# gareth-cross/mini_opt

Hardware: AMD Instinct MI355X
Metric: batched dense KKT Newton steps/sec, n=64 fp64 (higher is better)
Workload: dtype f64; 1 GPU; BASELINE configs[2]: batch=65536 per GPU, n=64 / 8 eq / 32 box, m_r=128, J-level input (row-major J), one mo_newton_step launch per step; mode=step, kernel=fused_mfma_f64_n64, batch_per_gpu=65536, batch_total=65536, n=64, k=8, m=32, m_r=128, parallelism=batch-sharded x1, no collectives

## Files before the change

### mini_opt_amd/csrc/kkt_fused.hip

```cpp
#include <math.h>
#include <stdlib.h>

#include <type_traits>

#include "mo_fused_select.h"

namespace mo {
namespace {

typedef double d2 __attribute__((ext_vector_type(2)));
typedef double d4 __attribute__((ext_vector_type(4)));

#ifdef MO_FUSED_STAMPS
#define MO_STAMP(i)                                                                                   \
  do {                                                                                                \
    __builtin_amdgcn_sched_barrier(0);                                                                \
    unsigned long long t__;                                                                           \
    asm volatile("s_memtime %0\n\ts_waitcnt lgkmcnt(0)" : "=s"(t__)::"memory");                       \
    stamp_acc[i] += t__ - stamp_prev;                                                                 \
    stamp_prev = t__;                                                                                 \
    __builtin_amdgcn_sched_barrier(0);                                                                \
  } while (0)
#else
#define MO_STAMP(i) do { } while (0)
// ... 188 lines not shown
        if (ta == tb && r > j) { row = 16 * ta + r; col = 16 * ta + j; }
        U[ta * NB + tb][t] = (row < nn && col < nn) ? G[row + (size_t)col * ld] : 0.0;
      }
    }
    cvec[ta] = (16 * ta + j < nn) ? cg[16 * ta + j] : 0.0;
  }
}

__device__ inline int lane_id() {
  int l;
  asm volatile("v_mbcnt_lo_u32_b32 %0, -1, 0\n\tv_mbcnt_hi_u32_b32 %0, -1, %0" : "=v"(l));
  return l;
}

typedef const KernelArgs __attribute__((address_space(4)))* KArgs;
__device__ inline KArgs fresh_args() {
  KArgs p = (KArgs)__builtin_amdgcn_kernarg_segment_ptr();
  asm volatile("" : "+s"(p));
  return p;
}

__device__ inline void dma16(const void* gsrc, unsigned lds_dst) {
  unsigned keep;
  asm volatile(
      "s_mov_b32 %0, m0\n\ts_mov_b32 m0, %2\n\ts_nop 0\n\tglobal_load_lds_dwordx4 %1, off\n\ts_mov_b32 m0, %0"
      : "=&s"(keep)
      : "v"(gsrc), "s"(lds_dst)
      : "memory");
}
__device__ inline const void* uniform_ptr(const void* p) {
  const unsigned long long b = (unsigned long long)(uintptr_t)p;
  const unsigned lo = __builtin_amdgcn_readfirstlane((unsigned)b), hi = __builtin_amdgcn_readfirstlane((unsigned)(b >> 32));
  return (const void*)(uintptr_t)(((unsigned long long)hi << 32) | lo);
}
#ifdef MO_J_NO_NT
#define MO_J_POLICY ""
#else
#define MO_J_POLICY " nt"
#endif
template <int IMM> __device__ inline void dma16_s(const void* sbase_in, unsigned voff, unsigned lds_dst_in) {
  const void* sbase = uniform_ptr(sbase_in);
  const unsigned lds_dst = __builtin_amdgcn_readfirstlane(lds_dst_in);
  unsigned keep;
  asm volatile(
      "s_mov_b32 %0, m0\n\ts_mov_b32 m0, %3\n\ts_nop 0\n\tglobal_load_lds_dwordx4 %1, %2 offset:%4" MO_J_POLICY "\n\ts_mov_b32 m0, %0"
      : "=&s"(keep)
      : "v"(voff), "s"(sbase), "s"(lds_dst), "i"(IMM)
      : "memory");
}
__device__ inline void dma4_s(const void* sbase_in, unsigned voff, unsigned lds_dst_in) {
  const void* sbase = uniform_ptr(sbase_in);
  const unsigned lds_dst = __builtin_amdgcn_readfirstlane(lds_dst_in);
  unsigned keep;
  asm volatile(
      "s_mov_b32 %0, m0\n\ts_mov_b32 m0, %3\n\ts_nop 0\n\tglobal_load_lds_dword %1, %2\n\ts_mov_b32 m0, %0"
      : "=&s"(keep)
      : "v"(voff), "s"(sbase), "s"(lds_dst)
      : "memory");
}
__device__ inline void dma4(const void* gsrc, unsigned lds_dst) {
  unsigned keep;
  asm volatile(
      "s_mov_b32 %0, m0\n\ts_mov_b32 m0, %2\n\ts_nop 0\n\tglobal_load_lds_dword %1, off\n\ts_mov_b32 m0, %0"
      : "=&s"(keep)
      : "v"(gsrc), "s"(lds_dst)
      : "memory");
}
__device__ inline void dma_doubles(const double* src, unsigned lds_dst, int count, int lane) {
  const unsigned voff = 4u * (unsigned)lane;
  if (lane < 2 * count) dma4_s(src, voff, lds_dst);
  if (lane + 64 < 2 * count) dma4_s(reinterpret_cast<const char*>(src) + 256, voff, lds_dst + 256);
  if (count > 64) {
    if (lane + 128 < 2 * count) dma4_s(reinterpret_cast<const char*>(src) + 512, voff, lds_dst + 512);
    if (lane + 192 < 2 * count) dma4_s(reinterpret_cast<const char*>(src) + 768, voff, lds_dst + 768);
  }
  if (count > 128) {
#pragma unroll
    for (int c = 4; c < 8; ++c)
      if (lane + 64 * c < 2 * count) dma4_s(reinterpret_cast<const char*>(src) + 256 * c, voff, lds_dst + 256 * c);
  }
}
template <int N> __device__ inline void wait_vmcnt() { asm volatile("s_waitcnt vmcnt(%0)" ::"i"(N) : "memory"); }
__device__ inline void lds_fence() { asm volatile("s_waitcnt lgkmcnt(0)" ::: "memory"); }

#ifdef MO_MASKED_PAD_4
#define MO_MASKED_PAD "4"
#else
#define MO_MASKED_PAD "0"
#endif
template <int LANE_IN_ROW> __device__ inline double row_bcast64(double v) {
  return __longlong_as_double(__builtin_amdgcn_mov_dpp(__double_as_longlong(v), 0x150 + LANE_IN_ROW, 0xf, 0xf, false));
}
template <unsigned long long MASK> __device__ inline void masked_set(double& dst, double src) {
  unsigned long long save;
  asm volatile("s_mov_b64 %[sv], exec\n\ts_mov_b32 exec_lo, %[lo]\n\ts_mov_b32 exec_hi, %[hi]\n\tv_mov_b64 %[d], %[s]\n\t"
               "s_mov_b64 exec, %[sv]\n\ts_nop " MO_MASKED_PAD
               : [d] "+v"(dst), [sv] "=&s"(save)
               : [s] "v"(src), [lo] "i"((unsigned)(MASK & 0xffffffffull)), [hi] "i"((unsigned)(MASK >> 32)));
}
template <unsigned long long MASK> __device__ inline void masked_set_neg(double& dst, double src) {
  unsigned long long save;
  asm volatile("s_mov_b64 %[sv], exec\n\ts_mov_b32 exec_lo, %[lo]\n\ts_mov_b32 exec_hi, %[hi]\n\tv_max_f64 %[d], -%[s], -%[s]\n\t"
               "s_mov_b64 exec, %[sv]\n\ts_nop " MO_MASKED_PAD
               : [d] "+v"(dst), [sv] "=&s"(save)
               : [s] "v"(src), [lo] "i"((unsigned)(MASK & 0xffffffffull)), [hi] "i"((unsigned)(MASK >> 32)));
}
template <unsigned long long MASK> __device__ inline void masked_zero4(d4& T) {
  unsigned long long save;
  double t0 = T[0], t1 = T[1], t2 = T[2], t3 = T[3];
  asm volatile(
      "s_mov_b64 %[sv], exec\n\ts_mov_b32 exec_lo, %[lo]\n\ts_mov_b32 exec_hi, %[hi]\n\tv_mov_b64 %[a], 0\n\tv_mov_b64 %[b], 0\n\t"
      "v_mov_b64 %[c], 0\n\tv_mov_b64 %[d], 0\n\ts_mov_b64 exec, %[sv]\n\ts_nop " MO_MASKED_PAD
      : [a] "+v"(t0), [b] "+v"(t1), [c] "+v"(t2), [d] "+v"(t3), [sv] "=&s"(save)
      : [lo] "i"((unsigned)(MASK & 0xffffffffull)), [hi] "i"((unsigned)(MASK >> 32)));
  T[0] = t0; T[1] = t1; T[2] = t2; T[3] = t3;
}
template <int K>
__device__ inline void sweep_step_lean(d4& T, double& bad, int g, int j) {
  constexpr int src_g = K & 3, src_t = K >> 2;
  constexpr unsigned long long mcol = 0x0001000100010001ull << K;
  constexpr unsigned long long mrow = 0xFFFFull << (16 * src_g);
  const double rowreg = T[src_t];
  const double d = readlane_f64(rowreg, 16 * src_g + K);
  double inv = __builtin_amdgcn_rcp(d);
  inv = fma(inv, fma(-d, inv, 1.0), inv);
  asm volatile("v_fma_f64 %0, %1, 0, %0" : "+v"(bad) : "v"(inv));
#ifdef MO_SWEEP_VALU_ROW
  double rk = bcast_from_row<src_g>(rowreg) * inv;
#else
  double rk = bpermute_f64((16 * src_g + j) * 4, rowreg) * inv;
#endif
  masked_set_neg<mcol>(rk, inv);
  double f[4];
#pragma unroll
  for (int t = 0; t < 4; ++t) f[t] = row_bcast64<K>(T[t]);
  masked_zero4<mcol>(T);
#pragma unroll
  for (int t = 0; t < 4; ++t) T[t] = fma(-f[t], rk, T[t]);
  double rowk_new = T[src_t];
  masked_set<mrow>(rowk_new, rk);
  T[src_t] = rowk_new;
}
template <int K, int KEND> struct SweepLoop {
  static __device__ inline void run(d4& T, double& bad, int npiv, int g, int j) {
    if (K < npiv) sweep_step_lean<K>(T, bad, g, j);
    SweepLoop<K + 1, KEND>::run(T, bad, npiv, g, j);
  }
};
template <int KEND> struct SweepLoop<KEND, KEND> {
  static __device__ inline void run(d4&, double&, int, int, int) {}
};
__device__ inline bool sweep_tile(d4& T, int npiv, int g, int j) {
  double bad = 0.0;
  SweepLoop<0, 16>::run(T, bad, npiv, g, j);
  return bad == 0.0;
}

template <int NT, int D, int JMODE = JMODE_VECTOR, int NY = 1, bool ROW0 = true>
struct JStream {
  static constexpr bool FLAT = JMODE == JMODE_FLAT, GATHER = JMODE == JMODE_GATHER;
  static constexpr int N = 16 * NT, NB = NT + NY, NH = NT / 2, NI = GATHER ? 2 * NT : (FLAT ? N / 8 : NH), DPS = NI + 1, SLOT = NH * 1024 + 64;
  static_assert((D - 1) * DPS <= 63, "vmcnt is a 6-bit counter");
  static_assert(D >= 2 && D <= 8, "ring depth");
  const char* jbase;
  const char* rbase;
  unsigned joff, roff;
  unsigned jstep;
  const double* tail_j; const double* tail_r; int rem, row_len, g_, j_;
  bool act0, act1, act2, act3;
  const char* lane_piece;
  const char* r_elem;
  unsigned ring_base;
  int lane, nsteps;
  long long rs_, cs_;

  __device__ inline void init(const double* Jp, const double* rg, const char* smem, unsigned ring_base_, int lane_, int g, int j, int m_r,
                              int nn = N, long long rs = -1, long long cs = 1) {
    if (rs < 0) rs = nn;
    jbase = reinterpret_cast<const char*>(Jp);
    rbase = reinterpret_cast<const char*>(rg);
    rs_ = 8 * rs; cs_ = 8 * cs;
    joff = GATHER ? (unsigned)(g * rs_ + 2 * j * cs_) : (unsigned)(g * nn + 2 * j) * 8u;
    jstep = GATHER ? (unsigned)(4 * rs_) : 32u * (unsigned)nn;
    act0 = 2 * j < nn; act1 = 32 + 2 * j < nn; act2 = 64 + 2 * j < nn; act3 = 96 + 2 * j < nn;
    roff = 4u * (unsigned)lane_;
    lane_piece = smem + lane_ * 16;
    r_elem = smem + NH * 1024 + 8 * g;
    ring_base = ring_base_; lane = lane_; nsteps = m_r >> 2;
    rem = m_r & 3; row_len = nn; g_ = g; j_ = j;
    tail_j = Jp + (size_t)(4 * nsteps) * (GATHER ? rs : (long long)nn); tail_r = rg + 4 * nsteps;
  }
  template <int IMM> __device__ static inline void dma4_si(const void* sbase_in, unsigned voff, unsigned lds_dst_in) {
    const void* sbase = uniform_ptr(sbase_in);
    const unsigned lds_dst = __builtin_amdgcn_readfirstlane(lds_dst_in);
    unsigned keep;
    asm volatile(
        "s_mov_b32 %0, m0\n\ts_mov_b32 m0, %3\n\ts_nop 0\n\tglobal_load_lds_dword %1, %2 offset:%4\n\ts_mov_b32 m0, %0"
        : "=&s"(keep)
        : "v"(voff), "s"(sbase), "s"(lds_dst), "i"(IMM)
        : "memory");
  }
  template <int SL> __device__ inline void issue() {
    const unsigned dst = ring_base + SL * SLOT;
    if (GATHER) {
#pragma unroll
      for (int c = 0; c < NT; ++c) {
        const int col0 = 32 * (c >> 1) + (c & 1);
        if (col0 < row_len) {
          const char* sb = jbase + (long long)col0 * cs_;
          if (col0 + 2 * j_ < row_len) { dma4_si<0>(sb, joff, dst + 512 * c); dma4_si<4>(sb, joff, dst + 512 * c + 256 - 4); }
        } else {
          if (lane == 0) { dma4_si<0>(jbase, 0u, dst + NH * 1024 + 48); dma4_si<0>(jbase, 0u, dst + NH * 1024 + 48); }
        }
      }
      if (lane < 8) dma4_s(rbase, roff, dst + NH * 1024);
      jbase += jstep;
      rbase += 32;
      return;
    }
    if (FLAT) {
      const int run = 32 * row_len;
#pragma unroll
      for (int i = 0; i < NI; ++i) {
        if (256 * i < run) {
          if (256 * i + 4 * lane < run) dma4_s(jbase + 256 * i, 4u * (unsigned)lane, dst + 256 * i);
        } else {
          if (lane == 0) dma4_s(jbase, 0u, dst + NH * 1024 + 48);
        }
      }
      if (lane < 8) dma4_s(rbase, roff, dst + NH * 1024);
      jbase += jstep;
      rbase += 32;
      return;
    }
    if (act0) dma16_s<0>(jbase, joff, dst);
    if (NH > 1 && act1) dma16_s<256>(jbase, joff, dst + 1024 - 256);
    if (NH > 2 && act2) dma16_s<512>(jbase, joff, dst + 2048 - 512);
    if (NH > 3 && act3) dma16_s<768>(jbase, joff, dst + 3072 - 768);
    if (lane < 8) dma4_s(rbase, roff, dst + NH * 1024);
    jbase += jstep;
    rbase += 32;
  }
  __device__ inline void wait_for_oldest(int younger) const {
    if (younger >= D - 1) { wait_vmcnt<(D - 1) * DPS>(); return; }
    switch (younger) {
      case 0: wait_vmcnt<0>(); break;
      case 1: wait_vmcnt<1 * DPS>(); break;
      case 2: wait_vmcnt<(D > 2 ? 2 : 0) * DPS>(); break;
      case 3: wait_vmcnt<(D > 3 ? 3 : 0) * DPS>(); break;
      case 4: wait_vmcnt<(D > 4 ? 4 : 0) * DPS>(); break;
      case 5: wait_vmcnt<(D > 5 ? 5 : 0) * DPS>(); break;
      default: wait_vmcnt<(D > 6 ? 6 : 0) * DPS>(); break;
    }
  }
  double rsq;
  template <int SL, bool RSQ = false> __device__ inline void consume(int q, d4 (&U)[NB * NB], double (&cpart)[NT]) {
    wait_for_oldest(nsteps - 1 - q);
    double ops[NT];
    if (GATHER) {
      const int* src = reinterpret_cast<const int*>(lane_piece - lane * 16 + SL * SLOT) + lane;
#pragma unroll
      for (int c = 0; c < NT; ++c) ops[c] = __hiloint2double(src[128 * c + 64], src[128 * c]);
    } else if (FLAT) {
      const double* src = reinterpret_cast<const double*>(lane_piece - lane * 16 + SL * SLOT) + g_ * row_len + 2 * j_;
#pragma unroll
      for (int h = 0; h < NH; ++h) {
        const double v0 = src[32 * h], v1 = src[32 * h + 1];
        ops[2 * h] = (32 * h + 2 * j_ < row_len) ? v0 : 0.0;
        ops[2 * h + 1] = (32 * h + 2 * j_ + 1 < row_len) ? v1 : 0.0;
      }
    } else {
#pragma unroll
      for (int h = 0; h < NH; ++h) {
        const d2 v = *(const d2*)(lane_piece + SL * SLOT + h * 1024);
        ops[2 * h] = v[0]; ops[2 * h + 1] = v[1];
      }
    }
    const double rq = *(const double*)(r_elem + SL * SLOT);
    lds_fence();
    if (q + D < nsteps) issue<SL>();
    if (RSQ) rsq = fma(rq, rq, rsq);
#pragma unroll
    for (int ta = 0; ta < NT; ++ta) {
      cpart[ta] = fma(ops[ta], rq, cpart[ta]);
#pragma unroll
      for (int tb = ta; tb < NT; ++tb) jtj_mfma(U[ta * NB + tb], ops[ta], ops[tb], ta);
    }
  }
#ifdef MO_ROW0_ALL_NY
  static constexpr bool ROW0_VGPR = NT == 8 && ROW0;
#elif !defined(MO_NO_ROW0_VGPR)
  static constexpr bool ROW0_VGPR = NT == 8 && NY == 1 && ROW0;
#else
  static constexpr bool ROW0_VGPR = false;
#endif
#ifndef MO_ROW0_ASM_QUAL
#define MO_ROW0_ASM_QUAL
#endif
#ifndef MO_ROW0_PREFIX
#define MO_ROW0_PREFIX "s_nop 3\n\t"
#endif
  __device__ static inline void jtj_mfma(d4& acc, double a, double b, int ta) {
    if (ROW0_VGPR && ta == 0) asm MO_ROW0_ASM_QUAL (MO_ROW0_PREFIX "v_mfma_f64_16x16x4_f64 %0, %1, %2, %0" : "+v"(acc) : "v"(a), "v"(b));
    else acc = __builtin_amdgcn_mfma_f64_16x16x4f64(a, b, acc, 0, 0, 0);
  }
  __device__ static inline void finish() {
    if (ROW0_VGPR) asm volatile("s_nop 15\n\ts_nop 3" ::: "memory");
  }
#define MO_FOR_SLOTS(F) F(0) F(1) F(2) F(3) F(4) F(5) F(6) F(7)
  __device__ inline void prologue() {
#define MO_ISSUE(u) if (u < D && u < nsteps) issue<(u < D ? u : 0)>();
    MO_FOR_SLOTS(MO_ISSUE)
#undef MO_ISSUE
  }
  template <bool RSQ = false>
  __device__ inline void run(d4 (&U)[NB * NB], double (&cpart)[NT]) {
    if (RSQ) rsq = 0.0;
    for (int q0 = 0; q0 < nsteps; q0 += D) {
#define MO_CONSUME(u) if (u < D && q0 + u < nsteps) consume<(u < D ? u : 0), RSQ>(q0 + u, U, cpart);
      MO_FOR_SLOTS(MO_CONSUME)
#undef MO_CONSUME
    }
    if (rem) {
      double ops[NT];
#pragma unroll
      for (int c = 0; c < NT; ++c) ops[c] = 0.0;
      double rq = 0.0;
      if (g_ < rem) {
        if (GATHER) {
          const char* row = reinterpret_cast<const char*>(tail_j) + g_ * rs_ + 2 * j_ * cs_;
#pragma unroll
          for (int c = 0; c < NT; ++c) {
            const int col0 = 32 * (c >> 1) + (c & 1);
            if (col0 + 2 * j_ < row_len) ops[c] = *reinterpret_cast<const double*>(row + (long long)col0 * cs_);
          }
        } else {
          const double* row = tail_j + (size_t)g_ * row_len + 2 * j_;
#pragma unroll
          for (int h = 0; h < NH; ++h) {
            if (32 * h + 2 * j_ < row_len) ops[2 * h] = row[32 * h];
            if (32 * h + 2 * j_ + 1 < row_len) ops[2 * h + 1] = row[32 * h + 1];
          }
        }
        rq = tail_r[g_];
      }
      if (RSQ) rsq = fma(rq, rq, rsq);
#pragma unroll
      for (int ta = 0; ta < NT; ++ta) {
        cpart[ta] = fma(ops[ta], rq, cpart[ta]);
#pragma unroll
        for (int tb = ta; tb < NT; ++tb) jtj_mfma(U[ta * NB + tb], ops[ta], ops[tb], ta);
      }
    }
    finish();
  }
#undef MO_FOR_SLOTS
};

template <int NT, int NY> __device__ inline int tile_pivots(int pa, int k) { return pa < NT + NY - 1 ? 16 : k - 16 * (NY - 1); }
template <int NT, int NY = 1>
__device__ inline bool block_eliminate(d4 (&U)[(NT + NY) * (NT + NY)], int k, int g, int j) {
  constexpr int NB = NT + NY;
  bool ok = true;
#pragma unroll
  for (int pa = 0; pa < NB; ++pa) {
    ok = sweep_tile(U[pa * NB + pa], tile_pivots<NT, NY>(pa, k), g, j) && ok;
    __builtin_amdgcn_sched_barrier(0);
#pragma unroll
    for (int pc = pa + 1; pc < NB; ++pc) {
      d4 negZ = mfma4(U[pa * NB + pa], U[pa * NB + pc], d4{0.0, 0.0, 0.0, 0.0});
#pragma unroll
      for (int pb = pa + 1; pb <= pc; ++pb) U[pb * NB + pc] = mfma4(U[pa * NB + pb], negZ, U[pb * NB + pc]);
      __builtin_amdgcn_sched_barrier(0);
    }
  }
  return ok;
}

#ifndef MO_LA_MIN_NT
#define MO_LA_MIN_NT 6
#endif
template <int NB> constexpr int la_count(int pa) { int c = 0; for (int pc = pa + 2; pc < NB; ++pc) c += 1 + (pc - pa); return c; }
template <int NB> constexpr int la_pc(int pa, int idx) {
  for (int pc = pa + 2; pc < NB; ++pc) { const int n = 1 + (pc - pa); if (idx < n) return pc; idx -= n; }
  return -1;
}
template <int NB> constexpr int la_sub(int pa, int idx) {
  for (int pc = pa + 2; pc < NB; ++pc) { const int n = 1 + (pc - pa); if (idx < n) return idx; idx -= n; }
  return -1;
}
template <int NT, int PA, int IDX, int Q> __device__ inline void la_mfma(d4 (&U)[(NT + 1) * (NT + 1)], d4& negZ) {
  constexpr int NB = NT + 1;
  if constexpr (IDX < la_count<NB>(PA)) {
    constexpr int pc = la_pc<NB>(PA, IDX), sub = la_sub<NB>(PA, IDX);
    if constexpr (sub == 0) {
      if constexpr (Q == 0) negZ = d4{0.0, 0.0, 0.0, 0.0};
      negZ = __builtin_amdgcn_mfma_f64_16x16x4f64(U[PA * NB + PA][Q], U[PA * NB + pc][Q], negZ, 0, 0, 0);
    } else {
      U[(PA + sub) * NB + pc] = __builtin_amdgcn_mfma_f64_16x16x4f64(U[PA * NB + (PA + sub)][Q], negZ[Q], U[(PA + sub) * NB + pc], 0, 0, 0);
    }
  }
}
template <int NB> constexpr int la_per_pivot(int pa) { return (la_count<NB>(pa) + 15) / 16; }
template <int NT, int PA, int K, int P> __device__ inline void la_point(d4 (&U)[(NT + 1) * (NT + 1)], d4& negZ) {
  constexpr int M = la_per_pivot<NT + 1>(PA);
  if constexpr (M <= 1) {
    la_mfma<NT, PA, K, P>(U, negZ);
  } else {
    constexpr int slot = M == 2 ? (P == 0 ? 0 : (P == 2 ? 1 : -1)) : (P < M ? P : -1);
    if constexpr (slot >= 0) {
      la_mfma<NT, PA, K * M + slot, 0>(U, negZ); la_mfma<NT, PA, K * M + slot, 1>(U, negZ);
      la_mfma<NT, PA, K * M + slot, 2>(U, negZ); la_mfma<NT, PA, K * M + slot, 3>(U, negZ);
    }
  }
}
template <int NT, int PA, int K>
__device__ inline void sweep_step_work(d4 (&U)[(NT + 1) * (NT + 1)], d4& negZ, double& bad, bool active, int g, int j) {
  constexpr int NB = NT + 1;
  constexpr int src_g = K & 3, src_t = K >> 2;
  constexpr unsigned long long mcol = 0x0001000100010001ull << K;
  constexpr unsigned long long mrow = 0xFFFFull << (16 * src_g);
  d4& T = U[(PA + 1) * NB + (PA + 1)];
  if (!active) {
    la_point<NT, PA, K, 0>(U, negZ); la_point<NT, PA, K, 1>(U, negZ); la_point<NT, PA, K, 2>(U, negZ); la_point<NT, PA, K, 3>(U, negZ);
    return;
  }
  const double rowreg = T[src_t];
  const double d = readlane_f64(rowreg, 16 * src_g + K);
  double inv = __builtin_amdgcn_rcp(d);
  const double rowk = bpermute_f64((16 * src_g + j) * 4, rowreg);
  __builtin_amdgcn_sched_barrier(0);
  la_point<NT, PA, K, 0>(U, negZ);
  __builtin_amdgcn_sched_barrier(0);
  inv = fma(inv, fma(-d, inv, 1.0), inv);
  asm volatile("v_fma_f64 %0, %1, 0, %0" : "+v"(bad) : "v"(inv));
// ... 74 lines not shown
    vt[0] = row_bcast64<kRC>(U[pa * NB + L][0]) - row_bcast64<0>(ws);
    vt[1] = row_bcast64<kRC>(U[pa * NB + L][1]) - row_bcast64<1>(ws);
    vt[2] = row_bcast64<kRC>(U[pa * NB + L][2]) - row_bcast64<2>(ws);
    vt[3] = row_bcast64<kRC>(U[pa * NB + L][3]) - row_bcast64<3>(ws);
    double q = 0.0;
#pragma unroll
    for (int t = 0; t < 4; ++t) q = fma(U[pa * NB + pa][t], vt[t], q);
    xb[pa] = -cross_row_sum(q);
    __builtin_amdgcn_sched_barrier(0);
  }
}

template <int NT, int NY = 1>
__device__ inline void solve_second_rhs(const d4 (&U)[(NT + NY) * (NT + NY)], int k, int g, int j, double (&rb)[NT + NY], double* hop,
                                        double* rbuf_x, double* rbuf_y, double (&xb)[NT + NY]) {
  constexpr int NB = NT + NY, L = NB - 1;
#pragma unroll
  for (int q = 0; q < NY; ++q) rb[NT + q] = (16 * q + j < k) ? rb[NT + q] : 0.0;
#pragma unroll
  for (int pa = 0; pa < NB; ++pa) {
    if (pa >= NT) rb[pa] = (16 * (pa - NT) + j < k) ? rb[pa] : 0.0;
    if (g == 0) { hop[j] = rb[pa]; (pa < NT ? rbuf_x + 16 * pa : rbuf_y + 16 * (pa - NT))[j] = rb[pa]; }
    lds_fence();
    if (pa < L) {
      double q = 0.0;
#pragma unroll
      for (int t = 0; t < 4; ++t) q = fma(U[pa * NB + pa][t], hop[g + 4 * t], q);
      const double w = cross_row_sum(q);
      lds_fence();
      if (g == 0) hop[j] = w;
      lds_fence();
      double wr[4];
#pragma unroll
      for (int t = 0; t < 4; ++t) wr[t] = hop[g + 4 * t];
#pragma unroll
      for (int pb = pa + 1; pb < NB; ++pb) {
        double q2 = 0.0;
#pragma unroll
        for (int t = 0; t < 4; ++t) q2 = fma(U[pa * NB + pb][t], wr[t], q2);
        rb[pb] += cross_row_sum(q2);
        if constexpr (NY >= 2) asm volatile("" : "+v"(rb[pb]));
      }
      lds_fence();
    }
  }
#pragma unroll
  for (int pa = L; pa >= 0; --pa) {
    const double* rsrc = pa < NT ? rbuf_x + 16 * pa : rbuf_y + 16 * (pa - NT);
    double vt[4], pt[4];
#pragma unroll
    for (int t = 0; t < 4; ++t) {
      pt[t] = 0.0;
#pragma unroll
      for (int pb = pa + 1; pb < NB; ++pb) pt[t] = fma(U[pa * NB + pb][t], xb[pb], pt[t]);
    }
    if (pa < L) {
      const double ws = row_sum4_scatter(pt[0], pt[1], pt[2], pt[3]);
      pt[0] = row_bcast64<0>(ws); pt[1] = row_bcast64<1>(ws); pt[2] = row_bcast64<2>(ws); pt[3] = row_bcast64<3>(ws);
    }
#pragma unroll
    for (int t = 0; t < 4; ++t) vt[t] = rsrc[g + 4 * t] - pt[t];
    double q = 0.0;
#pragma unroll
    for (int t = 0; t < 4; ++t) q = fma(U[pa * NB + pa][t], vt[t], q);
    xb[pa] = -cross_row_sum(q);
    if (pa >= NT) xb[pa] = (16 * (pa - NT) + j < k) ? xb[pa] : 0.0;
    __builtin_amdgcn_sched_barrier(0);
  }
}

template <int NT, int WPS, int MC = 1, int NY = 1, bool RHS = false> struct FusedCfg {
  static constexpr int N = 16 * NT;
  static constexpr int NH = NT / 2;
  static constexpr int DPS = NH + 1;
  static constexpr int SLOT = NH * 1024 + 64;
  static constexpr int MCAP = 64 * MC;
  static constexpr int VEC = (3 * N + 4 * MCAP + MCAP / 2 + 32 * NY + (RHS ? MCAP : 0)) * 8;
  static constexpr int D_FIT = ((160 * 1024) / (4 * WPS) - VEC) / SLOT;
  static constexpr int D_TUNED = NT > 4 ? 4 : (NT == 4 ? (WPS >= 3 ? 4 : 7) : (WPS >= 4 ? 4 : 8));
  static constexpr int D = MC == 1 ? D_TUNED : (D_FIT > 8 ? 8 : D_FIT);
  static_assert(D >= 2, "LDS budget");
  static constexpr int LDS = D * SLOT + VEC;
};

template <int NT, int WPS, bool QPL, int MC = 1, int JMODE = JMODE_VECTOR, int NY = 1, bool RHS = false>
__global__ __launch_bounds__(256 * WPS, WPS) void kkt_fused_f64_kernel(const KernelArgs a) {
  static_assert(!RHS || JMODE == JMODE_VECTOR, "the right-hand-side mode exists on the 16-byte stream and for (G, c) only");
  using C = FusedCfg<NT, WPS, MC, NY, RHS>;
  constexpr int MCAP = C::MCAP;
  constexpr int N = C::N, NB = NT + NY, LT = NB - 1, SLOT = C::SLOT, D = C::D;
  constexpr int WAVES = 4 * WPS;

  __shared__ __attribute__((aligned(16))) char smem_all[WAVES * C::LDS];
  const int wave = __builtin_amdgcn_readfirstlane((int)(threadIdx.x >> 6));
  char* const smem = smem_all + wave * C::LDS;
  double* const xs = reinterpret_cast<double*>(smem + D * SLOT);
  double* const diagS = xs + N;
  double* const rhsS = diagS + N;
  double* const rp = diagS;
  double* const dxs = rhsS;
  double* const cA = rhsS + N;
  double* const cB = cA + MCAP;
  double* const cS = cB + MCAP;
  double* const cZ = cS + MCAP;
  int* const cV = reinterpret_cast<int*>(cZ + MCAP);
  double* const yb = cZ + MCAP + MCAP / 2;
  double* const bb = yb + 16 * NY;
  double* const cP = bb + 16 * NY;
  const unsigned ring_base = (unsigned)(uintptr_t)smem;
  const unsigned vec_base = ring_base + D * SLOT;

  const int m_lay = a.m;
  const bool no_ineq = (a.flags & MO_STEP_NO_INEQUALITIES) != 0;
  const int k = a.k, m = no_ineq ? 0 : a.m, m_r = a.m_r;
  const int nn = a.n;
  const bool transpose = RHS && (a.flags & MO_KKT_TRANSPOSE) != 0;
  for (int i = (int)(threadIdx.x & 63); i < D * SLOT / 8; i += 64) reinterpret_cast<double*>(smem)[i] = 0.0;
  for (int i = (int)(threadIdx.x & 63); i < N; i += 64) xs[i] = 0.0;
  lds_fence();
#ifdef MO_FUSED_STAMPS
  unsigned long long stamp_acc[16] = {0, 0, 0, 0, 0, 0, 0, 0, 0, 0, 0, 0, 0, 0, 0, 0}, stamp_prev;
  asm volatile("s_memtime %0\n\ts_waitcnt lgkmcnt(0)" : "=s"(stamp_prev)::"memory");
  const unsigned long long stamp_t0 = stamp_prev, stamp_rt0 = __builtin_amdgcn_s_memrealtime();
#endif

  const int chunk_shift = 63 - __builtin_clzll((unsigned long long)gridDim.x * WAVES * 4);
  const long long waves_all = (long long)gridDim.x * WAVES;
  const bool st_rounds = a.static_rounds > 0 && a.batch <= (long long)a.static_rounds * waves_all;
  auto chunk_for = [&](long long observed) -> int {
    if (st_rounds) return 1;
    const long long c = (a.batch - observed) >> chunk_shift;
    return c < 1 ? 1 : (c > 8 ? 8 : (int)c);
  };
  auto take_ticket = [&](int chunk, long long p_now) -> unsigned long long {
    if (st_rounds) return (unsigned long long)p_now;
    unsigned long long t = 0;
    if (lane_id() == 0) t = atomicAdd(a.ticket, (unsigned long long)chunk);
    return t;
  };
  auto uniform64 = [](unsigned long long v) -> long long {
    const unsigned lo = __builtin_amdgcn_readfirstlane((unsigned)v), hi = __builtin_amdgcn_readfirstlane((unsigned)(v >> 32));
    return (long long)(((unsigned long long)hi << 32) | lo);
  };
  if (a.stagger > 0 && !st_rounds) {
    const int slot = wave >> 2;
    for (int i = 0; i < slot * a.stagger; ++i) __builtin_amdgcn_s_sleep(127);
  }
  int chunk = chunk_for(0);
  const long long ticket_base = (long long)gridDim.x * WAVES * chunk;
  long long p = st_rounds ? (long long)(wave >> 2) * ((long long)gridDim.x * 4) + (long long)blockIdx.x * 4 + (wave & 3) : ((long long)blockIdx.x * WAVES + wave) * chunk;
  long long chunk_end = p + chunk;

  while (p < a.batch) {
    const bool last_of_chunk = p + 1 >= chunk_end;
    int next_chunk = 0;
    unsigned long long next_ticket = 0;
    if (last_of_chunk) {
      next_chunk = chunk_for(p);
      next_ticket = take_ticket(next_chunk, p);
    }
    const int lane = lane_id();
    const int g = lane >> 4, j = lane & 15;

    const double* Jp = QPL ? nullptr : (const double*)a.J + p * a.J_stride;
    const double* rg = QPL ? nullptr : RHS ? Jp : (const double*)a.r + p * a.r_stride;
    KArgs ka = fresh_args();
    const double* vp = (const double*)ka->vars + p * ka->vars_stride;
    const double* gp = RHS ? (const double*)ka->rhs + p * ka->rhs_stride : nullptr;

    JStream<NT, D, JMODE, NY> stream;
    if (!QPL) {
      stream.init(Jp, rg, smem, ring_base, lane, g, j, m_r, nn, a.J_row_major ? (long long)a.J_ld : 1ll, a.J_row_major ? 1ll : (long long)a.J_ld);
      stream.prologue();
    }
    MO_STAMP(13);

    d4 U[NB * NB];
#pragma unroll
    for (int q = 0; q < NB * NB; ++q) U[q] = d4{0.0, 0.0, 0.0, 0.0};
    dma_doubles(RHS ? gp : vp, vec_base, nn, lane);
    if (m > 0) {
      const long long coff = p * ka->cons_stride;
      if (lane < m) dma4_s(ka->cons_var + coff, 4u * (unsigned)lane, vec_base + (3 * N + 4 * MCAP) * 8);
#pragma unroll
      for (int ci = 1; ci < MC; ++ci)
        if (lane + 64 * ci < m) dma4_s(ka->cons_var + coff + 64 * ci, 4u * (unsigned)lane, vec_base + (3 * N + 4 * MCAP) * 8 + 256 * ci);
      dma_doubles((const double*)ka->cons_a + coff, vec_base + (3 * N) * 8, m, lane);
      if (RHS) {
        dma_doubles(gp + nn, vec_base + (3 * N + MCAP) * 8, m, lane);
        dma_doubles(gp + nn + m + k, vec_base + (3 * N + 4 * MCAP + MCAP / 2 + 32 * NY) * 8, m, lane);
      } else {
        dma_doubles((const double*)ka->cons_b + coff, vec_base + (3 * N + MCAP) * 8, m, lane);
      }
      dma_doubles(vp + nn, vec_base + (3 * N + 2 * MCAP) * 8, m, lane);
      dma_doubles(vp + nn + m + k, vec_base + (3 * N + 3 * MCAP) * 8, m, lane);
    }
    if (k > 0) {
      if (!RHS) dma_doubles(vp + nn + m_lay, vec_base + (3 * N + 4 * MCAP + MCAP / 2) * 8, k, lane);
      dma_doubles(RHS ? gp + nn + m_lay : (const double*)ka->b + p * ka->b_stride, vec_base + (3 * N + 4 * MCAP + MCAP / 2 + 16 * NY) * 8, k, lane);
    }
    MO_STAMP(14);
    load_a_tiles<NT, QPL, NY>(k > 0 ? (const double*)ka->A + p * ka->A_stride : nullptr, ka->A_ld, k, nn, g, j, U);

    MO_STAMP(0);
    double cpart[NT];
#pragma unroll
    for (int c = 0; c < NT; ++c) cpart[c] = 0.0;
    double cvec[NT];
    if (QPL) {
      load_g_tiles<NT, NY>((const double*)ka->G + p * ka->G_stride, ka->G_ld, (const double*)ka->c + p * ka->c_stride, nn, g, j, U, cvec);
    } else {
#ifdef MO_FUSED_STAMPS
      stream.wait_for_oldest(stream.nsteps - 1);
      MO_STAMP(7);
#endif
      stream.run(U, cpart);
#pragma unroll
      for (int c = 0; c < NT; ++c) cvec[c] = cross_row_sum(cpart[c]);
    }
    MO_STAMP(1);

    wait_vmcnt<0>();
    ka = fresh_args();
    const double mu = ka->mu ? ((const double*)ka->mu)[p * ka->mu_stride] : 0.0;
    if (lane < N / 2) {
      diagS[2 * lane] = 0.0; diagS[2 * lane + 1] = 0.0;
      rhsS[2 * lane] = 0.0; rhsS[2 * lane + 1] = 0.0;
    }
    int cvar[MC]; double ca[MC], cb[MC], cs[MC], cz[MC], cs_inv[MC];
    double cp[MC];
    bool bad_index[MC];
#pragma unroll
    for (int ci = 0; ci < MC; ++ci) {
      const int ix = lane + 64 * ci;
      cvar[ci] = 0; ca[ci] = 1.0; cb[ci] = 0.0; cs[ci] = 1.0; cz[ci] = 0.0; cp[ci] = 0.0;
      if (ix < m) { cvar[ci] = cV[ix]; ca[ci] = cA[ix]; cb[ci] = cB[ix]; cs[ci] = cS[ix]; cz[ci] = cZ[ix]; }
      if (RHS && ix < m) {
        cp[ci] = cP[ix];
        if (transpose) { cb[ci] = -(cs[ci] * cb[ci]); cB[ix] = cb[ci]; }
      }
    }
    lds_fence();
    bool lane_bad_slack = false, lane_bad_index = false;
#pragma unroll
    for (int ci = 0; ci < MC; ++ci) {
      const int ix = lane + 64 * ci;
      bad_index[ci] = (ix < m) && ((cvar[ci] < 0) || (cvar[ci] >= nn));
      if (bad_index[ci]) cvar[ci] = 0;
      lane_bad_index = lane_bad_index || bad_index[ci];
      lane_bad_slack = lane_bad_slack || ((ix < m) && !(cs[ci] > 0.0));
      cs_inv[ci] = rcp_f64(cs[ci]);
      if (ix < m) {
        const double zs = cz[ci] * cs_inv[ci];
        atomicAdd(&diagS[cvar[ci]], ca[ci] * zs * ca[ci]);
        if (RHS) atomicAdd(&rhsS[cvar[ci]], -(ca[ci] * (cb[ci] + cz[ci] * cp[ci]) * cs_inv[ci]));
        else atomicAdd(&rhsS[cvar[ci]], ca[ci] * (cz[ci] * (cs[ci] - cb[ci]) + mu) * cs_inv[ci]);
      }
    }
    const bool slack_bad = __any(lane_bad_slack);
    bool any_bad_index = __any(lane_bad_index);
    if (no_ineq && m_lay > 0) {
      bool bad = false;
      const int* cvp = ka->cons_var + p * ka->cons_stride;
      for (int ix = lane; ix < m_lay; ix += 64) { const int v = cvp[ix]; bad = bad || v < 0 || v >= nn; }
      any_bad_index = __any(bad);
    }
    lds_fence();
    double dS[NT], rS[NT];
    ldv<NT, QPL>(diagS, j, dS);
    ldv<NT, QPL>(rhsS, j, rS);
    if (RHS) {
      double rd[NT];
      ldv<NT, QPL>(xs, j, rd);
#pragma unroll
      for (int c = 0; c < NT; ++c) cvec[c] = transpose ? -rd[c] : rd[c];
    }
    if (g == 0) {
#pragma unroll
      for (int c = 0; c < NT; ++c) rp[16 * c + j] = rS[c] - cvec[c];
    }
    lds_fence();

#pragma unroll
    for (int t = 0; t < 4; ++t) {
      constexpr int e0 = 16 * (NY - 1);
      double v = 0.0;
      if (j == kRC) v = (e0 + g + 4 * t < k) ? -bb[e0 + g + 4 * t] : 0.0;
      if (g + 4 * t == kRC) v = (e0 + j < k) ? -bb[e0 + j] : 0.0;
      U[LT * NB + LT][t] = v;
#pragma unroll
      for (int q = 0; q < NY - 1; ++q) {
        if (j == kRC) U[(NT + q) * NB + LT][t] = -bb[16 * q + g + 4 * t];
      }
    }
    const double lam_in = ka->lambda_vec ? ((const double*)ka->lambda_vec)[p * ka->lambda_vec_stride] : ka->lambda;
    const double lam = (!QPL && lam_in > 0.0) ? lam_in : 0.0;
    double padv[NT];
    pad_diag<NT, QPL>(j, nn, padv);
#pragma unroll
    for (int c = 0; c < NT; ++c) {
#pragma unroll
      for (int t = 0; t < 4; ++t) {
        U[c * NB + c][t] += (j == g + 4 * t) ? (lam + dS[c] + padv[c]) : 0.0;
        const double rv = rp[16 * c + g + 4 * t];
        if (j == kRC) U[c * NB + LT][t] = rv;
      }
    }

    MO_STAMP(2);
    __builtin_amdgcn_sched_barrier(0);
    if (a.chain_prio) __builtin_amdgcn_s_setprio(1);
    bool ok = true;
    constexpr bool kLookAhead = NT >= MO_LA_MIN_NT && NY == 1;
    if constexpr (kLookAhead) {
      ok = block_eliminate_lookahead<NT>(U, k, g, j);
    } else {
#pragma unroll
    for (int pa = 0; pa < NB; ++pa) {
      ok = sweep_tile(U[pa * NB + pa], tile_pivots<NT, NY>(pa, k), g, j) && ok;
      __builtin_amdgcn_sched_barrier(0);
      MO_STAMP(3);
#pragma unroll
      for (int pc = pa + 1; pc < NB; ++pc) {
        d4 negZ = mfma4(U[pa * NB + pa], U[pa * NB + pc], d4{0.0, 0.0, 0.0, 0.0});
#pragma unroll
        for (int pb = pa + 1; pb <= pc; ++pb) U[pb * NB + pc] = mfma4(U[pa * NB + pb], negZ, U[pb * NB + pc]);
        __builtin_amdgcn_sched_barrier(0);
      }
      MO_STAMP(4);
    }
    }

    __builtin_amdgcn_sched_barrier(0);
    double xb[NB];
    back_substitute<NT, NY>(U, k, j, xb);

    MO_STAMP(5);
    ka = fresh_args();
    double dxv[NT];
    {
      double xn[NT];
      if (!RHS) ldv<NT, QPL>(xs, j, xn);
#pragma unroll
      for (int c = 0; c < NT; ++c) dxv[c] = RHS ? xb[c] : xb[c] - xn[c];
    }
    bool finite = true;
#pragma unroll
    for (int c = 0; c < NT; ++c) finite = finite && (fabs(dxv[c]) < INFINITY);
    if (g == 0) stv<NT, QPL>(dxs, j, dxv);
    lds_fence();
    double dsv[MC], dzv[MC], ap = 1.0, ad = 1.0;
#pragma unroll
    for (int ci = 0; ci < MC; ++ci) {
      const int ix = lane + 64 * ci;
      dsv[ci] = 0.0; dzv[ci] = 0.0;
      if (ix < m) {
        const double ca2 = cA[ix], cb2 = cB[ix], cs2 = cS[ix], cz2 = cZ[ix];
        const int cvar2 = bad_index[ci] ? 0 : cV[ix];
        const double csi = MC == 1 ? cs_inv[ci] : rcp_f64(cs2);
        if (RHS) {
          dsv[ci] = ca2 * dxs[cvar2] + cP[ix];
          dzv[ci] = -(cb2 + cz2 * dsv[ci]) * csi;
          finite = finite && (fabs(dsv[ci]) < INFINITY) && (fabs(dzv[ci]) < INFINITY);
          if (transpose) { dsv[ci] *= csi; dzv[ci] = -dzv[ci]; }
          continue;
        }
        const double r_pi = ca2 * xs[cvar2] + cb2 - cs2;
        dsv[ci] = ca2 * dxs[cvar2] + r_pi;
        dzv[ci] = -(cz2 * csi) * dsv[ci] - csi * (cs2 * cz2 - mu);
        const double tau = ka->tau;
        if (cs2 + dsv[ci] <= 0.0 && fabs(dsv[ci]) > 0.0) ap = fmin(ap, -tau * cs2 * rcp_f64(dsv[ci]));
        if (cz2 + dzv[ci] <= 0.0 && fabs(dzv[ci]) > 0.0) ad = fmin(ad, -tau * cz2 * rcp_f64(dzv[ci]));
        finite = finite && (fabs(dsv[ci]) < INFINITY) && (fabs(dzv[ci]) < INFINITY);
      }
    }
    if (!RHS) {
      ap = cross_row_min(row_min(ap));
      ad = cross_row_min(row_min(ad));
    }
    double dyv[NY];
#pragma unroll
    for (int q = 0; q < NY; ++q) {
      if (RHS) dyv[q] = (16 * q + j < k) ? (transpose ? xb[NT + q] : -xb[NT + q]) : 0.0;
      else dyv[q] = (16 * q + j < k) ? (-xb[NT + q] - yb[16 * q + j]) : 0.0;
      finite = finite && (fabs(dyv[q]) < INFINITY);
    }
    int st = MO_STATUS_OK;
    if (!__all(finite)) st = MO_STATUS_NONFINITE;
    if (!ok) st = MO_STATUS_FACTORIZATION_FAILED;
    if (slack_bad) st = MO_STATUS_NONPOSITIVE_SLACK;
    if (any_bad_index) st = MO_STATUS_BAD_INDEX;
    const double nanv = __builtin_nan("");
    double* dp = (double*)ka->delta + p * ka->delta_stride;
    if (g == 0) {
      double outv[NT];
#pragma unroll
      for (int c = 0; c < NT; ++c) outv[c] = st == MO_STATUS_OK ? dxv[c] : nanv;
      stv_n<NT, QPL>(dp, j, nn, outv);
#pragma unroll
      for (int q = 0; q < NY; ++q)
        if (16 * q + j < k) dp[nn + m_lay + 16 * q + j] = st == MO_STATUS_OK ? dyv[q] : nanv;
    }
    if (no_ineq) {
      for (int ix = lane; ix < m_lay; ix += 64) { dp[nn + ix] = st == MO_STATUS_OK ? 0.0 : nanv; dp[nn + m_lay + k + ix] = st == MO_STATUS_OK ? 0.0 : nanv; }
    }
#pragma unroll
    for (int ci = 0; ci < MC; ++ci) {
      const int ix = lane + 64 * ci;
      if (ix < m) {
        dp[nn + ix] = st == MO_STATUS_OK ? dsv[ci] : nanv;
        dp[nn + m + k + ix] = st == MO_STATUS_OK ? dzv[ci] : nanv;
      }
    }
    if (lane == 0) {
      if (!RHS && ka->alpha) {
        ((double*)ka->alpha)[2 * p] = st == MO_STATUS_OK ? ap : nanv;
        ((double*)ka->alpha)[2 * p + 1] = st == MO_STATUS_OK ? ad : nanv;
      }
      if (ka->status) ka->status[p] = st;
    }
    lds_fence();
    if (a.chain_prio) __builtin_amdgcn_s_setprio(0);
    MO_STAMP(6);
    if (last_of_chunk) {
      p = uniform64(next_ticket) + ticket_base;
      chunk_end = p + next_chunk;
    } else {
      ++p;
    }
  }
#ifdef MO_FUSED_STAMPS
  if ((threadIdx.x & 63) == 0 && a.debug) {
    for (int i = 0; i < 8; ++i) atomicAdd(a.debug + i, stamp_acc[i]);
    atomicAdd(a.debug + 13, stamp_acc[13]); atomicAdd(a.debug + 14, stamp_acc[14]);
    atomicAdd(a.debug + 8, 1ull);
    const unsigned long long life = stamp_prev - stamp_t0, rt = __builtin_amdgcn_s_memrealtime() - stamp_rt0;
    atomicMax(a.debug + 9, life);
    atomicMin(a.debug + 10, life);
    atomicAdd(a.debug + 11, rt);
    atomicMax(a.debug + 12, rt);
  }
#endif
}

template <int NT, int WPS, int JMODE = JMODE_VECTOR>
__global__ __launch_bounds__(256 * WPS, WPS) void kkt_fused_linearize_kernel(const KernelArgs a) {
  using C = FusedCfg<NT, WPS>;
  constexpr int NB = NT + 1, SLOT = C::SLOT, D = C::D;
  constexpr int WAVES = 4 * WPS;
  __shared__ __attribute__((aligned(16))) char smem_all[WAVES * C::LDS];
  const int wave = __builtin_amdgcn_readfirstlane((int)(threadIdx.x >> 6));
  char* const smem = smem_all + wave * C::LDS;
  const unsigned ring_base = (unsigned)(uintptr_t)smem;
  const int nn = a.n, m_r = a.m_r;
  for (int i = (int)(threadIdx.x & 63); i < D * SLOT / 8; i += 64) reinterpret_cast<double*>(smem)[i] = 0.0;
  lds_fence();
  const int chunk_shift = 63 - __builtin_clzll((unsigned long long)gridDim.x * WAVES * 4);
  const long long waves_all = (long long)gridDim.x * WAVES;
  const bool st_rounds = a.static_rounds > 0 && a.batch <= (long long)a.static_rounds * waves_all;
  auto chunk_for = [&](long long observed) -> int {
    if (st_rounds) return 1;
    const long long c = (a.batch - observed) >> chunk_shift;
    return c < 1 ? 1 : (c > 8 ? 8 : (int)c);
  };
  auto take_ticket = [&](int chunk, long long p_now) -> unsigned long long {
    if (st_rounds) return (unsigned long long)p_now;
    unsigned long long t = 0;
    if (lane_id() == 0) t = atomicAdd(a.ticket, (unsigned long long)chunk);
    return t;
  };
  auto uniform64 = [](unsigned long long v) -> long long {
    const unsigned lo = __builtin_amdgcn_readfirstlane((unsigned)v), hi = __builtin_amdgcn_readfirstlane((unsigned)(v >> 32));
    return (long long)(((unsigned long long)hi << 32) | lo);
  };
  int chunk = chunk_for(0);
  const long long ticket_base = (long long)gridDim.x * WAVES * chunk;
  long long p = st_rounds ? (long long)(wave >> 2) * ((long long)gridDim.x * 4) + (long long)blockIdx.x * 4 + (wave & 3) : ((long long)blockIdx.x * WAVES + wave) * chunk;
  long long chunk_end = p + chunk;
  while (p < a.batch) {
    const bool last_of_chunk = p + 1 >= chunk_end;
    int next_chunk = 0;
    unsigned long long next_ticket = 0;
    if (last_of_chunk) { next_chunk = chunk_for(p); next_ticket = take_ticket(next_chunk, p); }
    const int lane = lane_id();
    const int g = lane >> 4, j = lane & 15;
    JStream<NT, D, JMODE> stream;
    stream.init((const double*)a.J + p * a.J_stride, (const double*)a.r + p * a.r_stride, smem, ring_base, lane, g, j, m_r, nn,
                a.J_row_major ? (long long)a.J_ld : 1ll, a.J_row_major ? 1ll : (long long)a.J_ld);
    stream.prologue();
    d4 U[NB * NB];
#pragma unroll
    for (int q = 0; q < NB * NB; ++q) U[q] = d4{0.0, 0.0, 0.0, 0.0};
    double cpart[NT];
#pragma unroll
    for (int c = 0; c < NT; ++c) cpart[c] = 0.0;
    stream.template run<true>(U, cpart);
    double cvec[NT];
#pragma unroll
    for (int c = 0; c < NT; ++c) cvec[c] = cross_row_sum(cpart[c]);
    const double half_sq = 0.5 * cross_row_sum(stream.rsq);
    const double lam_in = a.lambda_vec ? ((const double*)a.lambda_vec)[p * a.lambda_vec_stride] : a.lambda;
    const double lam = lam_in > 0.0 ? lam_in : 0.0;
// ... 942 lines not shown
```

Measured before the change: 51.12 million steps/s.

## Software-pipeline J stream operand loads and peel first MFMA step to zero-init

Adds a pipelined JStream mode that loads the next step's operands from LDS while the current step's MFMAs run, alternating two operand register sets. It also peels the first step so the J^T J accumulators start from a literal-zero MFMA instead of being explicitly zeroed. A lean path restructures the diagonal/rhs setup and the output-writing NaN selection into branch-hoisted forms. These target LDS-latency stalls and redundant VALU work, at the cost of doubling operand register pressure, which could lower occupancy or cause spills. The mode is enabled by default for NT<=4, single-MC, non-QPL, non-RHS configurations.

Result: no change. 51.13 million steps/s, median of 2 (+0.0%).

```diff
diff --git a/mini_opt_amd/csrc/kkt_fused.hip b/mini_opt_amd/csrc/kkt_fused.hip
--- a/mini_opt_amd/csrc/kkt_fused.hip
+++ b/mini_opt_amd/csrc/kkt_fused.hip
@@ -294,6 +294,11 @@
 }
 template <int N> __device__ inline void wait_vmcnt() { asm volatile("s_waitcnt vmcnt(%0)" ::"i"(N) : "memory"); }
 __device__ inline void lds_fence() { asm volatile("s_waitcnt lgkmcnt(0)" ::: "memory"); }
+__device__ inline void lds_fence_counted() {
+  asm volatile("" ::: "memory");
+  __builtin_amdgcn_s_waitcnt(0xC07F);
+  asm volatile("" ::: "memory");
+}
 
 #ifdef MO_MASKED_PAD_4
 #define MO_MASKED_PAD "4"
@@ -368,9 +373,11 @@
   return bad == 0.0;
 }
 
-template <int NT, int D, int JMODE = JMODE_VECTOR, int NY = 1, bool ROW0 = true>
+constexpr int STREAM_PIPE = 1, STREAM_PEEL = 2;
+template <int NT, int D, int JMODE = JMODE_VECTOR, int NY = 1, bool ROW0 = true, int OPT = 0>
 struct JStream {
   static constexpr bool FLAT = JMODE == JMODE_FLAT, GATHER = JMODE == JMODE_GATHER;
+  static constexpr bool PIPE = (OPT & STREAM_PIPE) != 0, PEEL = (OPT & STREAM_PEEL) != 0;
   static constexpr int N = 16 * NT, NB = NT + NY, NH = NT / 2, NI = GATHER ? 2 * NT : (FLAT ? N / 8 : NH), DPS = NI + 1, SLOT = NH * 1024 + 64;
   static_assert((D - 1) * DPS <= 63, "vmcnt is a 6-bit counter");
   static_assert(D >= 2 && D <= 8, "ring depth");
@@ -466,9 +473,7 @@
     }
   }
   double rsq;
-  template <int SL, bool RSQ = false> __device__ inline void consume(int q, d4 (&U)[NB * NB], double (&cpart)[NT]) {
-    wait_for_oldest(nsteps - 1 - q);
-    double ops[NT];
+  template <int SL> __device__ inline void load_ops(double (&ops)[NT], double& rq) const {
     if (GATHER) {
       const int* src = reinterpret_cast<const int*>(lane_piece - lane * 16 + SL * SLOT) + lane;
 #pragma unroll
@@ -488,16 +493,36 @@
         ops[2 * h] = v[0]; ops[2 * h + 1] = v[1];
       }
     }
-    const double rq = *(const double*)(r_elem + SL * SLOT);
+    rq = *(const double*)(r_elem + SL * SLOT);
+  }
+  template <bool RSQ, bool ZC> __device__ inline void products(const double (&ops)[NT], double rq, d4 (&U)[NB * NB], double (&cpart)[NT]) {
+    if (RSQ) rsq = fma(rq, rq, rsq);
+#pragma unroll
+    for (int ta = 0; ta < NT; ++ta) {
+      cpart[ta] = fma(ops[ta], rq, cpart[ta]);
+#pragma unroll
+      for (int tb = ta; tb < NT; ++tb) jtj_mfma<ZC>(U[ta * NB + tb], ops[ta], ops[tb], ta);
+    }
+  }
+  template <int SL, bool RSQ = false> __device__ inline void consume(int q, d4 (&U)[NB * NB], double (&cpart)[NT]) {
+    wait_for_oldest(nsteps - 1 - q);
+    double ops[NT], rq;
+    load_ops<SL>(ops, rq);
     lds_fence();
     if (q + D < nsteps) issue<SL>();
-    if (RSQ) rsq = fma(rq, rq, rsq);
-#pragma unroll
-    for (int ta = 0; ta < NT; ++ta) {
-      cpart[ta] = fma(ops[ta], rq, cpart[ta]);
-#pragma unroll
-      for (int tb = ta; tb < NT; ++tb) jtj_mfma(U[ta * NB + tb], ops[ta], ops[tb], ta);
-    }
+    products<RSQ, false>(ops, rq, U, cpart);
+  }
+  static_assert(!PIPE || D % 2 == 0, "the operand sets alternate with the slots");
+  template <int SL, bool RSQ, bool ZC>
+  __device__ inline void consume_pipe(int q, d4 (&U)[NB * NB], double (&cpart)[NT], const double (&ops)[NT], const double& rq, double (&nops)[NT],
+                                      double& nrq) {
+    lds_fence_counted();
+    if (q + D < nsteps) issue<SL>();
+    if (q + 1 < nsteps) {
+      wait_for_oldest(nsteps - 2 - q);
+      load_ops<(SL + 1) % D>(nops, nrq);
+    }
+    products<RSQ, ZC>(ops, rq, U, cpart);
   }
 #ifdef MO_ROW0_ALL_NY
   static constexpr bool ROW0_VGPR = NT == 8 && ROW0;
@@ -512,8 +537,10 @@
 #ifndef MO_ROW0_PREFIX
 #define MO_ROW0_PREFIX "s_nop 3\n\t"
 #endif
-  __device__ static inline void jtj_mfma(d4& acc, double a, double b, int ta) {
-    if (ROW0_VGPR && ta == 0) asm MO_ROW0_ASM_QUAL (MO_ROW0_PREFIX "v_mfma_f64_16x16x4_f64 %0, %1, %2, %0" : "+v"(acc) : "v"(a), "v"(b));
+  static_assert(!(PEEL && ROW0_VGPR), "the row-0 assembly MFMA accumulates in place: no literal-zero form");
+  template <bool ZC = false> __device__ static inline void jtj_mfma(d4& acc, double a, double b, int ta) {
+    if (ZC) acc = __builtin_amdgcn_mfma_f64_16x16x4f64(a, b, d4{0.0, 0.0, 0.0, 0.0}, 0, 0, 0);
+    else if (ROW0_VGPR && ta == 0) asm MO_ROW0_ASM_QUAL (MO_ROW0_PREFIX "v_mfma_f64_16x16x4_f64 %0, %1, %2, %0" : "+v"(acc) : "v"(a), "v"(b));
     else acc = __builtin_amdgcn_mfma_f64_16x16x4f64(a, b, acc, 0, 0, 0);
   }
   __device__ static inline void finish() {
@@ -525,44 +552,79 @@
     MO_FOR_SLOTS(MO_ISSUE)
 #undef MO_ISSUE
   }
+  __device__ inline void load_tail(double (&ops)[NT], double& rq) const {
+#pragma unroll
+    for (int c = 0; c < NT; ++c) ops[c] = 0.0;
+    rq = 0.0;
+    if (g_ < rem) {
+      const double* const tj = OPT ? reinterpret_cast<const double*>(jbase) : tail_j;
+      const double* const tr = OPT ? reinterpret_cast<const double*>(rbase) : tail_r;
+      if (GATHER) {
+        const char* row = reinterpret_cast<const char*>(tj) + g_ * rs_ + 2 * j_ * cs_;
+#pragma unroll
+        for (int c = 0; c < NT; ++c) {
+          const int col0 = 32 * (c >> 1) + (c & 1);
+          if (col0 + 2 * j_ < row_len) ops[c] = *reinterpret_cast<const double*>(row + (long long)col0 * cs_);
+        }
+      } else {
+        const double* row = tj + (size_t)g_ * row_len + 2 * j_;
+#pragma unroll
+        for (int h = 0; h < NH; ++h) {
+          if (32 * h + 2 * j_ < row_len) ops[2 * h] = row[32 * h];
+          if (32 * h + 2 * j_ + 1 < row_len) ops[2 * h + 1] = row[32 * h + 1];
+        }
+      }
+      rq = tr[g_];
+    }
+    if (OPT) {
+#pragma unroll
+      for (int c = 0; c < NT; ++c) asm volatile("" : "+v"(ops[c]));
+      asm volatile("" : "+v"(rq));
+    }
+  }
   template <bool RSQ = false>
   __device__ inline void run(d4 (&U)[NB * NB], double (&cpart)[NT]) {
     if (RSQ) rsq = 0.0;
+    bool tail_done = false;
+    if (PIPE || PEEL) {
+      double ops0[NT], rq0, ops1[NT], rq1;
+      if (nsteps > 0) {
+        wait_for_oldest(nsteps - 1);
+        load_ops<0>(ops0, rq0);
+      } else if (PEEL) {
+        load_tail(ops0, rq0);
+        tail_done = true;
+      }
+      if (PEEL || nsteps > 0) {
+        if (PIPE) {
+          consume_pipe<0, RSQ, PEEL>(0, U, cpart, ops0, rq0, ops1, rq1);
+        } else {
+          lds_fence();
+          if (D < nsteps) issue<0>();
+          products<RSQ, PEEL>(ops0, rq0, U, cpart);
+        }
+      }
+      for (int q0 = 1; q0 < nsteps; q0 += D) {
+#define MO_CONSUME(u)                                                                                      \
+  if (u < D && q0 + u < nsteps) {                                                                          \
+    if (PIPE && u % 2 == 0) consume_pipe<(u < D ? (u + 1) % D : 0), RSQ, false>(q0 + u, U, cpart, ops1, rq1, ops0, rq0);      \
+    else if (PIPE) consume_pipe<(u < D ? (u + 1) % D : 0), RSQ, false>(q0 + u, U, cpart, ops0, rq0, ops1, rq1);              \
+    else consume<(u < D ? (u + 1) % D : 0), RSQ>(q0 + u, U, cpart);                                        \
+  }
+        MO_FOR_SLOTS(MO_CONSUME)
+#undef MO_CONSUME
+      }
+    } else {
     for (int q0 = 0; q0 < nsteps; q0 += D) {
 #define MO_CONSUME(u) if (u < D && q0 + u < nsteps) consume<(u < D ? u : 0), RSQ>(q0 + u, U, cpart);
       MO_FOR_SLOTS(MO_CONSUME)
 #undef MO_CONSUME
     }
-    if (rem) {
-      double ops[NT];
-#pragma unroll
-      for (int c = 0; c < NT; ++c) ops[c] = 0.0;
-      double rq = 0.0;
-      if (g_ < rem) {
-        if (GATHER) {
-          const char* row = reinterpret_cast<const char*>(tail_j) + g_ * rs_ + 2 * j_ * cs_;
-#pragma unroll
-          for (int c = 0; c < NT; ++c) {
-            const int col0 = 32 * (c >> 1) + (c & 1);
-            if (col0 + 2 * j_ < row_len) ops[c] = *reinterpret_cast<const double*>(row + (long long)col0 * cs_);
-          }
-        } else {
-          const double* row = tail_j + (size_t)g_ * row_len + 2 * j_;
-#pragma unroll
-          for (int h = 0; h < NH; ++h) {
-            if (32 * h + 2 * j_ < row_len) ops[2 * h] = row[32 * h];
-            if (32 * h + 2 * j_ + 1 < row_len) ops[2 * h + 1] = row[32 * h + 1];
-          }
-        }
-        rq = tail_r[g_];
-      }
-      if (RSQ) rsq = fma(rq, rq, rsq);
-#pragma unroll
-      for (int ta = 0; ta < NT; ++ta) {
-        cpart[ta] = fma(ops[ta], rq, cpart[ta]);
-#pragma unroll
-        for (int tb = ta; tb < NT; ++tb) jtj_mfma(U[ta * NB + tb], ops[ta], ops[tb], ta);
-      }
+    }
+    if (rem && !tail_done) {
+      double ops[NT], rq;
+      load_tail(ops, rq);
+      products<RSQ, false>(ops, rq, U, cpart);
     }
     finish();
   }
@@ -803,6 +865,15 @@
   static_assert(D >= 2, "LDS budget");
   static constexpr int LDS = D * SLOT + VEC;
 };
+
+constexpr int step_stream_opt(int NT, int WPS, bool QPL, int MC, int JMODE, int NY, bool RHS) {
+  if (QPL || NT > 4 || MC != 1 || NY != 1 || RHS) return 0;
+#ifdef MO_STREAM_OPT
+  return MO_STREAM_OPT;
+#else
+  return STREAM_PIPE | STREAM_PEEL;
+#endif
+}
 
 template <int NT, int WPS, bool QPL, int MC = 1, int JMODE = JMODE_VECTOR, int NY = 1, bool RHS = false>
 __global__ __launch_bounds__(256 * WPS, WPS) void kkt_fused_f64_kernel(const KernelArgs a) {
@@ -889,7 +960,13 @@
     const double* vp = (const double*)ka->vars + p * ka->vars_stride;
     const double* gp = RHS ? (const double*)ka->rhs + p * ka->rhs_stride : nullptr;
 
-    JStream<NT, D, JMODE, NY> stream;
+    constexpr int kStreamOpt = step_stream_opt(NT, WPS, QPL, MC, JMODE, NY, RHS);
+#ifdef MO_NO_STEP_LEAN
+    constexpr bool kLean = false;
+#else
+    constexpr bool kLean = kStreamOpt != 0;
+#endif
+    JStream<NT, D, JMODE, NY, true, kStreamOpt> stream;
     if (!QPL) {
       stream.init(Jp, rg, smem, ring_base, lane, g, j, m_r, nn, a.J_row_major ? (long long)a.J_ld : 1ll, a.J_row_major ? 1ll : (long long)a.J_ld);
       stream.prologue();
@@ -898,23 +975,27 @@
 
     d4 U[NB * NB];
 #pragma unroll
-    for (int q = 0; q < NB * NB; ++q) U[q] = d4{0.0, 0.0, 0.0, 0.0};
+    for (int q = 0; q < NB * NB; ++q) {
+      if (!((kStreamOpt & STREAM_PEEL) && q / NB < NT && q % NB < NT)) U[q] = d4{0.0, 0.0, 0.0, 0.0};
+    }
     dma_doubles(RHS ? gp : vp, vec_base, nn, lane);
     if (m > 0) {
+      int md = m;
+      if (kStreamOpt) asm volatile("" : "+s"(md));
       const long long coff = p * ka->cons_stride;
       if (lane < m) dma4_s(ka->cons_var + coff, 4u * (unsigned)lane, vec_base + (3 * N + 4 * MCAP) * 8);
 #pragma unroll
       for (int ci = 1; ci < MC; ++ci)
         if (lane + 64 * ci < m) dma4_s(ka->cons_var + coff + 64 * ci, 4u * (unsigned)lane, vec_base + (3 * N + 4 * MCAP) * 8 + 256 * ci);
-      dma_doubles((const double*)ka->cons_a + coff, vec_base + (3 * N) * 8, m, lane);
+      dma_doubles((const double*)ka->cons_a + coff, vec_base + (3 * N) * 8, md, lane);
       if (RHS) {
-        dma_doubles(gp + nn, vec_base + (3 * N + MCAP) * 8, m, lane);
-        dma_doubles(gp + nn + m + k, vec_base + (3 * N + 4 * MCAP + MCAP / 2 + 32 * NY) * 8, m, lane);
+        dma_doubles(gp + nn, vec_base + (3 * N + MCAP) * 8, md, lane);
+        dma_doubles(gp + nn + m + k, vec_base + (3 * N + 4 * MCAP + MCAP / 2 + 32 * NY) * 8, md, lane);
       } else {
-        dma_doubles((const double*)ka->cons_b + coff, vec_base + (3 * N + MCAP) * 8, m, lane);
-      }
-      dma_doubles(vp + nn, vec_base + (3 * N + 2 * MCAP) * 8, m, lane);
-      dma_doubles(vp + nn + m + k, vec_base + (3 * N + 3 * MCAP) * 8, m, lane);
+        dma_doubles((const double*)ka->cons_b + coff, vec_base + (3 * N + MCAP) * 8, md, lane);
+      }
+      dma_doubles(vp + nn, vec_base + (3 * N + 2 * MCAP) * 8, md, lane);
+      dma_doubles(vp + nn + m + k, vec_base + (3 * N + 3 * MCAP) * 8, md, lane);
     }
     if (k > 0) {
       if (!RHS) dma_doubles(vp + nn + m_lay, vec_base + (3 * N + 4 * MCAP + MCAP / 2) * 8, k, lane);
@@ -1018,6 +1099,22 @@
     const double lam = (!QPL && lam_in > 0.0) ? lam_in : 0.0;
     double padv[NT];
     pad_diag<NT, QPL>(j, nn, padv);
+    if constexpr (kLean) {
+#pragma unroll
+      for (int t = 0; t < 4; ++t) {
+        if (j == g + 4 * t) {
+#pragma unroll
+          for (int c = 0; c < NT; ++c) U[c * NB + c][t] += lam + dS[c] + padv[c];
+        }
+      }
+      if (j == kRC) {
+#pragma unroll
+        for (int c = 0; c < NT; ++c) {
+#pragma unroll
+          for (int t = 0; t < 4; ++t) U[c * NB + LT][t] = rp[16 * c + g + 4 * t];
+        }
+      }
+    } else {
 #pragma unroll
     for (int c = 0; c < NT; ++c) {
 #pragma unroll
@@ -1026,6 +1123,7 @@
         const double rv = rp[16 * c + g + 4 * t];
         if (j == kRC) U[c * NB + LT][t] = rv;
       }
+    }
     }
 
     MO_STAMP(2);
@@ -1113,6 +1211,42 @@
     if (any_bad_index) st = MO_STATUS_BAD_INDEX;
     const double nanv = __builtin_nan("");
     double* dp = (double*)ka->delta + p * ka->delta_stride;
+    if constexpr (kLean) {
+      double zero = 0.0;
+      if (st != MO_STATUS_OK) {
+#pragma unroll
+        for (int c = 0; c < NT; ++c) dxv[c] = nanv;
+#pragma unroll
+        for (int q = 0; q < NY; ++q) dyv[q] = nanv;
+#pragma unroll
+        for (int ci = 0; ci < MC; ++ci) { dsv[ci] = nanv; dzv[ci] = nanv; }
+        ap = nanv; ad = nanv; zero = nanv;
+      }
+      if (g == 0) {
+        stv_n<NT, QPL>(dp, j, nn, dxv);
+#pragma unroll
+        for (int q = 0; q < NY; ++q)
+          if (16 * q + j < k) dp[nn + m_lay + 16 * q + j] = dyv[q];
+      }
+      if (no_ineq) {
+        for (int ix = lane; ix < m_lay; ix += 64) { dp[nn + ix] = zero; dp[nn + m_lay + k + ix] = zero; }
+      }
+#pragma unroll
+      for (int ci = 0; ci < MC; ++ci) {
+        const int ix = lane + 64 * ci;
+        if (ix < m) {
+          dp[nn + ix] = dsv[ci];
+          dp[nn + m + k + ix] = dzv[ci];
+        }
+      }
+      if (lane == 0) {
+        if (!RHS && ka->alpha) {
+          ((double*)ka->alpha)[2 * p] = ap;
+          ((double*)ka->alpha)[2 * p + 1] = ad;
+        }
+        if (ka->status) ka->status[p] = st;
+      }
+    } else {
     if (g == 0) {
       double outv[NT];
 #pragma unroll
@@ -1139,6 +1273,7 @@
         ((double*)ka->alpha)[2 * p + 1] = st == MO_STATUS_OK ? ad : nanv;
       }
       if (ka->status) ka->status[p] = st;
+    }
     }
     lds_fence();
     if (a.chain_prio) __builtin_amdgcn_s_setprio(0);
```
